# wangg12/mx-DeepIM

Measured on AMD Instinct MI355X. Metric: pose-refinements/sec (4 iters, 480x640), higher is better.
Workload: dtype f32

## Files before the change

### include/deepim_hip.h

```cpp
#ifndef DEEPIM_HIP_H_
#define DEEPIM_HIP_H_

#ifdef __cplusplus
extern "C" {
#endif

#define DIM_OK 0
#define DIM_ERR_ARG (-1)
#define DIM_ERR_LAUNCH (-2)
#define DIM_STATUS_OBS_BOX_EMPTY 1
#define DIM_STATUS_REN_BOX_EMPTY 2
#define DIM_STATUS_BAD_CLASS 4
#define DIM_STATUS_BAD_FACE 8
#define DIM_STATUS_BAD_K 16
#define DIM_STATUS_ICP_FEW_POINTS 32
#define DIM_STATUS_HYP_NO_SCORE 64
#define DIM_STATUS_FLOW_PNP_FEW_POINTS 128
#define DIM_STATUS_LAYER_HIDDEN 256
#define DIM_STATUS_COARSE_BAD_BOX 512
#define DIM_STATUS_PHOTO_FEW_POINTS 1024
#define DIM_STATUS_SIL_FEW_POINTS 2048
#define DIM_STATUS_TRACK_LOST 4096
#define DIM_STATUS_TRACK_REINIT 8192
#define DIM_STATUS_TRACK_OCCLUDED 16384
// ... 239 lines not shown

int dim_modelnet_light_position(const float* poses, float dx, float dy, float dz, float* light_pos, int B, void* stream);
int dim_box_mask(const int* bbox, float* mask, int B, int H, int W, int* bbox_of_mask, void* stream);

long dim_scene_compose_workspace_bytes(int N, int S, int H, int W);
int dim_scene_compose(const float* layer_bgr, const float* layer_depth, const int* layer_label, int N, int S, int H, int W,
                      void* workspace, float* scene_bgr, float* scene_depth, float* scene_label, float* vis_mask, int* counts,
                      int* vis_bbox, int* status, void* stream);

long dim_conv2d_packed_weight_floats(int Cout, int Cin, int KH, int KW);
int dim_conv2d_pack_weight(const float* w_oihw, float* w_packed, int Cout, int Cin, int KH, int KW, void* stream);
long dim_conv2d_workspace_floats(int N, int H, int W, int Cin, int Cout, int KH, int KW, int stride, int pad, int splits);
int dim_conv2d_fwd(const float* x, const float* w_packed, const float* bias, float* y, float* workspace, int N, int H, int W,
                   int Cin, int Cout, int KH, int KW, int stride, int pad, float slope, int splits, int tile, void* stream);
int dim_conv2d_fwd_partial(const float* x, const float* w_packed, float* workspace, int N, int H, int W, int Cin, int Cout, int KH,
                           int KW, int stride, int pad, int splits, int tile, void* stream);
int dim_splitk_reduce(const float* slabs, const float* bias, float* y, long M, int Cout, int splits, float slope, void* stream);
int dim_conv2d_tail_plan(int M, int Cout, int Cin, int KH, int KW, int tile, int* tail_begin_tile, int* tail_splits);
int dim_conv_auto_plan(long M, int Cout, int nchunks, int cin, int* tile, int* splits);
int dim_winograd_gemm_tile(int Cout, long tiles);
int dim_winograd_gemm_tile_planes(int Cout, long tiles, int planes);
int dim_set_winograd_split(int on);
int dim_get_winograd_split(void);
long dim_winograd_plane_gemm_weight_floats(int K, int Cout, int P);
int dim_winograd_plane_gemm_split_weights(float* U_packed, int K, int Cout, int P, void* stream);
int dim_winograd_plane_gemm(const float* V, const float* U_packed, float* M, int T, int K, int Cout, int P, int tile, int* used_split,
                            void* stream);
int dim_conv2d_fwd_ex(const float* x, const float* w_packed, const float* bias, float* y, int N, int H, int W, int Cin, int in_cstride,
                      int Cout, int KH, int KW, int stride, int pad, float slope, int tile, int out_cstride, int out_coff, int OH,
                      int OW, int osy, int osx, int ooy, int oox, int Ho, int Wo, int pad_w, int accumulate, void* stream);

long dim_winograd_packed_weight_floats(int Cout, int Cin, int m);
long dim_winograd_workspace_floats(int N, int H, int W, int Cin, int Cout, int m);
int dim_winograd_pack_weight(const float* w_oihw, float* w_packed, int Cout, int Cin, int m, void* stream);
int dim_winograd_dgrad_pack_weight(const float* w_oihw, float* w_packed, int Cout, int Cin, int m, void* stream);
int dim_conv2d_fwd_winograd(const float* x, const float* w_packed, const float* bias, float* y, float* workspace, int N, int H, int W,
                            int Cin, int in_cstride, int Cout, int out_cstride, int out_coff, float slope, int tile, int m,
                            void** events4, void* stream);
long dim_winograd5x5s2_packed_weight_floats(int Cout, int Cin);
long dim_winograd5x5s2_workspace_floats(int N, int H, int W, int Cin, int Cout);
int dim_winograd5x5s2_pack_weight(const float* w_oihw, float* w_packed, int Cout, int Cin, void* stream);
int dim_conv2d_fwd_winograd5x5s2(const float* x, const float* w_packed, const float* bias, float* y, float* workspace, int N, int H, int W,
                                 int Cin, int in_cstride, int Cout, int out_cstride, int out_coff, float slope, int tile, void** events4,
                                 void* stream);
int dim_wino_item_map_create(void** map, int N, int H, int W, int Cin, int Cout, int tile);
void dim_wino_item_map_destroy(void* map);
// ... 176 lines not shown
```

### mx-deepim_amd/csrc/common.h

```cpp
#pragma once
#include <hip/hip_runtime.h>
#include <cstdarg>
#include <cstdio>
#include <cstdint>
#include <utility>

#include "../../include/deepim_hip.h"

namespace dim {

constexpr int kWave = 64;

char* err_buf();
int set_err(int code, const char* fmt, ...);

inline hipStream_t as_stream(void* s) { return reinterpret_cast<hipStream_t>(s); }

inline int check_launch(const char* what) {
  hipError_t e = hipGetLastError();
  if (e != hipSuccess) return set_err(DIM_ERR_LAUNCH, "%s: %s", what, hipGetErrorString(e));
  return DIM_OK;
}

inline int ceil_div(long a, long b) { return (int)((a + b - 1) / b); }
// ... 177 lines not shown
int conv2d_unpack_weight_slabs(const float* w_packed, int nslab, long slab_stride, float* w_oihw, int Cout, int CoutPad, int Cin, int KH, int KW,
                               float scale, int accumulate, void* stream);

struct WGemmArgs {
  const float* V;
  const float* U;
  float* M;
  int T, K, Cout, P;
  int nch;
  int NTN;
  int per, rem;
  unsigned v_bytes, u_bytes, m_bytes;
  FastDiv d_nch, d_P, d_NTN, d_MT;
  int G, BM, BN, tile;
  int MT;
  int plane_major;
  int dbg_plain;
  int wide_flush;
  const void* U3;
  unsigned u3_bytes;
  int split;
  int skip5, q;
  const int* sigma;
};
inline long wino_packed_with_split(long u_floats) { return u_floats + (u_floats * 3 + 1) / 2; }
int wino_split_weights(float* U, long chunks, int Cout, hipStream_t st);
void wino_set_split(int on);
int wino_get_split();
bool wino_gemm_split_has(int tile);
int wino_gemm_split_slots(int tile);
int wino_gemm_split_run(const WGemmArgs& a, hipStream_t st);
int wino_gemm_plan(WGemmArgs* plan, const float* V, const float* U, float* M, int T, int K, int Cout, int P, int tile, int skip5 = 0);
void wino_tile_shape(int* tile, int Cout, int* BM, int* BN);
enum { kMapT, kMapK, kMapCout, kMapTile, kMapG, kMapPer, kMapRem, kMapLiveBefore, kMapLiveAfter, kMapMoved, kMapItems, kMapNch, kMapWords };
struct WinoItemMap {
  int hdr[kMapWords];
  int* host;
  int* dev;
};
int wino_item_map_build(int T, int K, int Cout, int tile, int G, int skip5, int* hdr, int** table);
inline const int* wino_item_map_for(const WinoItemMap* m, const WGemmArgs& a) {
  if (!m || !m->dev || !a.split || !a.skip5) return nullptr;
  const int* h = m->hdr;
  return (h[kMapT] == a.T && h[kMapK] == a.K && h[kMapCout] == a.Cout && h[kMapTile] == a.tile && h[kMapG] == a.G && h[kMapPer] == a.per &&
          h[kMapRem] == a.rem) ? m->dev : nullptr;
}
int wino_gemm_run(const WGemmArgs& plan, bool zeroed, hipStream_t st);

#ifdef __HIPCC__
struct WCur {
  int ch, p, nt, mt;
  int m;
// ... 123 lines not shown
```

### mx-deepim_amd/csrc/conv.hip

```cpp
#include "conv_impl.h"

namespace dim {

__global__ void splitk_reduce_kernel(const float* __restrict__ slabs, const float* __restrict__ bias, float* __restrict__ y,
                                     long MC, int Cout, int splits, float slope, int has_bias) {
  long i4 = (long)blockIdx.x * blockDim.x + threadIdx.x;
  long i = i4 * 4;
  if (i >= MC) return;
  float4 s = *reinterpret_cast<const float4*>(slabs + i);
  for (int k = 1; k < splits; ++k) {
    float4 p = *reinterpret_cast<const float4*>(slabs + (long)k * MC + i);
    s.x += p.x; s.y += p.y; s.z += p.z; s.w += p.w;
  }
  if (has_bias) {
    int c = (int)(i % Cout);
    s.x += bias[c]; s.y += bias[c + 1]; s.z += bias[c + 2]; s.w += bias[c + 3];
  }
  s.x = s.x > 0.f ? s.x : s.x * slope;
  s.y = s.y > 0.f ? s.y : s.y * slope;
  s.z = s.z > 0.f ? s.z : s.z * slope;
  s.w = s.w > 0.f ? s.w : s.w * slope;
  *reinterpret_cast<float4*>(y + i) = s;
}

// ... 84 lines not shown
  auto best_split = [&](long tiles, int smax) {
    double best = 1e30;
    int bs = 1;
    for (int s = 1; s <= smax; ++s) {
      if (!(s * 4 <= nchunks || s == 1)) continue;
      const double t = (double)((tiles * s + n_cu - 1) / n_cu) / s + 0.02 * s;
      if (t < best) { best = t; bs = s; }
    }
    return bs;
  };
  const bool wide = Cout % 128 == 0 && cin != 8;
  const long tiles = wide ? (M + 127) / 128 * (Cout / 128) : (M + 63) / 64 * (Cout / 64);
  *tile = wide ? 4 : 3;
  *splits = tiles >= n_cu ? 0 : best_split(tiles, 8);
  return DIM_OK;
}

int dim_set_winograd_split(int on) {
  wino_set_split(on ? 1 : 0);
  return DIM_OK;
}
int dim_get_winograd_split(void) { return wino_get_split(); }

static bool plane_gemm_on_device(const void* p) {
  hipPointerAttribute_t at;
  const hipError_t e = hipPointerGetAttributes(&at, p);
  if (e != hipSuccess) (void)hipGetLastError();
  return e == hipSuccess && (at.type == hipMemoryTypeDevice || at.type == hipMemoryTypeManaged);
}
long dim_winograd_plane_gemm_weight_floats(int K, int Cout, int P) {
  if (K <= 0 || Cout <= 0 || P <= 0) return 0;
  return wino_packed_with_split((long)P * K * Cout);
}
int dim_winograd_plane_gemm_split_weights(float* U_packed, int K, int Cout, int P, void* stream) {
  DIM_REQUIRE(K > 0 && K % 32 == 0 && Cout > 0 && Cout % 64 == 0 && P > 0, "winograd plane gemm: K %% 32 == 0 and Cout %% 64 == 0 required");
  DIM_REQUIRE(U_packed, "null pointer");
  DIM_REQUIRE(plane_gemm_on_device(U_packed), "winograd plane gemm: U_packed is not a device pointer");
  return wino_split_weights(U_packed, (long)P * (K / 32), Cout, as_stream(stream));
}
int dim_winograd_plane_gemm(const float* V, const float* U_packed, float* M, int T, int K, int Cout, int P, int tile, int* used_split,
                            void* stream) {
  DIM_REQUIRE(T > 0 && K > 0 && K % 32 == 0 && Cout > 0 && Cout % 64 == 0 && P > 0,
              "winograd plane gemm: T, P > 0, K %% 32 == 0 and Cout %% 64 == 0 required");
  DIM_REQUIRE(V && U_packed && M && used_split, "null pointer");
  DIM_REQUIRE(plane_gemm_on_device(V) && plane_gemm_on_device(U_packed) && plane_gemm_on_device(M),
              "winograd plane gemm: V, U_packed and M must be device pointers");
  WGemmArgs plan;
  const int rc = wino_gemm_plan(&plan, V, U_packed, M, T, K, Cout, P, tile);
  if (rc != DIM_OK) return rc;
  *used_split = plan.split;
  return wino_gemm_run(plan, false, as_stream(stream));
}

int dim_winograd_gemm_tile_planes(int Cout, long tiles, int planes) {
  static const int bn256 = [] { const char* e = getenv("DIM_WINO_BN256"); return e ? atoi(e) : 1; }();
  static const int fewrow = [] { const char* e = getenv("DIM_WINO_FEWROW"); return e ? atoi(e) : 1; }();
  if (Cout % 128) return 3;
  if (tiles < 1024) {
    if (!fewrow) return 3;
    if (wino_get_split()) {
      const struct { int tile, bm; double eff; } cand[2] = {{4, 128, 1.0}, {7, 96, planes > 36 ? 0.75 : 0.85}};
      const int cus = 256, slots = 512;
      int best = 7;
      double best_cost = 1e30;
      for (const auto& c : cand) {
        const long items = (tiles + c.bm - 1) / c.bm * (Cout / 128) * planes;
        long G = items < slots ? items : slots;
        if (G > cus && G < slots) G = G / cus * cus;
        const double cost = (double)items / (double)G * c.bm / c.eff;
        if (cost < best_cost) { best_cost = cost; best = c.tile; }
      }
      return best;
    }
    const struct { int tile, bm; double eff; } cand[3] = {{3, 64, 0.54}, {7, 96, 0.70}, {6, 160, 0.74}};
    int best = 3;
    double best_cost = 1e30;
    for (const auto& c : cand) {
      const double cost = (double)((tiles + c.bm - 1) / c.bm * c.bm) / c.eff;
      if (cost < best_cost) { best_cost = cost; best = c.tile; }
    }
    return best;
  }
  static const int big = [] { const char* e = getenv("DIM_WINO_BIG_TILE"); return e ? atoi(e) : 0; }();
  if (big == 6 || big == 7) return big;
  return (Cout % 256 == 0 && bn256) ? 5 : 4;
}
int dim_winograd_gemm_tile(int Cout, long tiles) { return dim_winograd_gemm_tile_planes(Cout, tiles, 36); }

// ... 359 lines not shown
```

### mx-deepim_amd/csrc/wino_gemm.hip

```cpp
#include <cstdlib>

#include "common.h"

namespace dim {

typedef float f32x16 __attribute__((ext_vector_type(16)));

__device__ __forceinline__ void wcur_advance(WCur& c, const WGemmArgs& a) {
  if (a.plane_major) return wcur_advance_pm(c, a);
  if (++c.ch == a.nch) {
    c.ch = 0;
    if (a.plane_major) {
      if (++c.nt == a.NTN) {
        c.nt = 0;
        if (++c.mt == a.MT) {
          c.mt = 0;
          ++c.p;
        }
      }
    } else if (++c.p == a.P) {
      c.p = 0;
      if (++c.nt == a.NTN) {
        c.nt = 0;
        ++c.mt;
// ... 180 lines not shown
    W_MFMA_GROUP(1, SET, 3)                                                            \
    buf ^= 1;                                                                          \
    W_FLUSH_CHECK(KCUR)                                                                \
  }
  int buf = 0;
  for (int kc = c_begin; kc < c_end; kc += 2) {
    W_CHUNK_BODY(0, kc)
    if (kc + 1 < c_end) W_CHUNK_BODY(1, kc + 1)
  }
#undef W_CHUNK_BODY
#undef W_FLUSH_CHECK
#undef W_MFMA_GROUP
#undef W_LOAD_BFRAG
#undef W_FRAG_READ
#undef W_STORE_CHUNK
#undef W_LOAD_CHUNK
}

__global__ __launch_bounds__(256) void wino_gemm_zero_kernel(WGemmArgs a) { wino_gemm_zero_tile(a, blockIdx.x + 1); }

static int g_wino_split = getenv("DIM_WINO_SPLIT") ? atoi(getenv("DIM_WINO_SPLIT")) : 1;
void wino_set_split(int on) { g_wino_split = on; }
int wino_get_split() { return g_wino_split; }
static int g_wino_cus = 0;
template <int BM, int BN, int WM, int WN>
static int wino_gemm_slots() {
  static int slots = 0;
  if (slots == 0) {
    int dev = 0, cus = 0, occ = 0;
    hipError_t e = hipGetDevice(&dev);
    if (e == hipSuccess) e = hipDeviceGetAttribute(&cus, hipDeviceAttributeMultiprocessorCount, dev);
    if (e == hipSuccess)
      e = hipOccupancyMaxActiveBlocksPerMultiprocessor(&occ, reinterpret_cast<const void*>(&wino_gemm_kernel<BM, BN, WM, WN>),
                                                       WM * WN * 64, (2 * BM * 36 + WM * WN * 512) * sizeof(float));
    if (e != hipSuccess || cus <= 0 || occ <= 0) return set_err(DIM_ERR_LAUNCH, "winograd gemm occupancy query: %s", hipGetErrorString(e));
    slots = cus * occ;
    g_wino_cus = cus;
  }
  return slots;
}

void wino_tile_shape(int* tile, int Cout, int* BM, int* BN) {
  if (*tile == 5 && Cout % 256 != 0) *tile = 4;
  if ((*tile < 4 || *tile > 7) || Cout % 128 != 0) *tile = 3;
  *BM = *tile == 3 ? 64 : *tile == 6 ? 160 : *tile == 7 ? 96 : 128;
  *BN = *tile == 5 ? 256 : *tile == 3 ? 64 : 128;
// ... 18 lines not shown
  a.P = P;
  a.nch = K / 32;
  a.NTN = Cout / BN;
  a.v_bytes = (unsigned)((long)T * P * K * 4);
  a.u_bytes = (unsigned)((long)P * K * Cout * 4);
  a.m_bytes = (unsigned)((long)T * P * Cout * 4);
  a.d_nch = make_fastdiv((unsigned)a.nch);
  a.d_P = make_fastdiv((unsigned)P);
  a.d_NTN = make_fastdiv((unsigned)a.NTN);
  a.MT = (int)MT;
  a.d_MT = make_fastdiv((unsigned)MT);
  static const int order = getenv("DIM_WINO_PLANE_MAJOR") ? atoi(getenv("DIM_WINO_PLANE_MAJOR")) : 1;
  a.plane_major = order;
  static const int dbg_plain = getenv("DIM_WINO_DBG_PLAIN") ? atoi(getenv("DIM_WINO_DBG_PLAIN")) : 0;
  a.dbg_plain = dbg_plain;
  static const int wide = getenv("DIM_WINO_WIDE_FLUSH") ? atoi(getenv("DIM_WINO_WIDE_FLUSH")) : 1;
  a.wide_flush = wide;
  a.BM = BM;
  a.BN = BN;
  a.tile = tile;
  a.split = g_wino_split && wino_gemm_split_has(tile) && (long)P * K * Cout * 6 < (1L << 31);
  a.U3 = U + (long)P * K * Cout;
  a.u3_bytes = (unsigned)((long)P * K * Cout * 6);
  DIM_REQUIRE(!skip5 || (P == 36 && a.nch % 4 == 0), "winograd gemm: skipping zero phase blocks needs 36 planes and K = 4 phases of whole chunks");
  a.skip5 = skip5;
  a.q = a.nch / 4;
  if (a.split || skip5) a.plane_major = 1;
  const int slots = a.split ? wino_gemm_split_slots(tile) : tile == 5 ? wino_gemm_slots<128, 256, 2, 4>() : tile == 4 ? wino_gemm_slots<128, 128, 2, 4>()
                  : tile == 6 ? wino_gemm_slots<160, 128, 1, 4>() : tile == 7 ? wino_gemm_slots<96, 128, 1, 4>() : wino_gemm_slots<64, 64, 2, 2>();
  if (slots <= 0) return slots;
  a.G = items < slots ? (int)items : slots;
  static const int g_round = getenv("DIM_WINO_G_ROUND") ? atoi(getenv("DIM_WINO_G_ROUND")) : 1;
  if (g_wino_cus == 0) {
    int dev = 0;
    if (hipGetDevice(&dev) != hipSuccess || hipDeviceGetAttribute(&g_wino_cus, hipDeviceAttributeMultiprocessorCount, dev) != hipSuccess) g_wino_cus = 0;
  }
  if (g_round && g_wino_cus > 0 && a.G > g_wino_cus && a.G < slots) a.G = a.G / g_wino_cus * g_wino_cus;
  if (const char* e = getenv("DIM_WINO_MAX_G")) {
    const int cap = atoi(e);
    if (cap > 0 && cap < a.G) a.G = cap;
  }
  const long total = items * a.nch;
  a.per = (int)(total / a.G);
  a.rem = (int)(total % a.G);
  *plan = a;
  return DIM_OK;
// ... 29 lines not shown
```

### mx-deepim_amd/csrc/wino_gemm_split.hip

```cpp
#include <cstdlib>

#include "common.h"

#ifndef DIM_SPLIT_EXP
#define DIM_SPLIT_EXP 0
#endif
#ifndef DIM_SPLIT_OPT
#define DIM_SPLIT_OPT 0
#endif

namespace dim {

typedef float f32x16 __attribute__((ext_vector_type(16)));
typedef float f32x4 __attribute__((ext_vector_type(4)));
typedef __bf16 bf16x8 __attribute__((ext_vector_type(8)));
typedef __bf16 bf16x4 __attribute__((ext_vector_type(4)));

struct Split4 {
  uint2 h, m, l;
};
__device__ __forceinline__ Split4 split3(const float4 v) {
  const f32x4 x = {v.x, v.y, v.z, v.w};
  const bf16x4 bh = __builtin_convertvector(x, bf16x4);
  const f32x4 r1 = x - __builtin_convertvector(bh, f32x4);
// ... 31 lines not shown
                     make_fastdiv((unsigned)Cout));
  return check_launch("winograd_split_weights");
}

#if DIM_SPLIT_EXP & 128
__device__ unsigned long long g_split_stamps[1024 * 8 * 11];
#endif
#if (DIM_SPLIT_EXP & 128) && defined(__HIP_DEVICE_COMPILE__)
#define S_STAMP(K)                                                                     \
  {                                                                                    \
    unsigned long long t_;                                                             \
    __builtin_amdgcn_sched_barrier(0);                                                 \
    asm volatile("s_memtime %0\n\ts_waitcnt lgkmcnt(0)" : "=s"(t_)::"memory");         \
    __builtin_amdgcn_sched_barrier(0);                                                 \
    seg[K] += t_ - tprev;                                                              \
    tprev = t_;                                                                        \
  }
#else
#define S_STAMP(K)
#endif

__device__ __forceinline__ void wscur_advance(WCur& c, const WGemmArgs& a, const WTab& t) { wcur_advance_pm(c, a, t); }

template <int BM, int WN, bool TAB>
__device__ __forceinline__ void wino_gemm_split_body(const WGemmArgs& a) {
  constexpr int BK = 32;
  constexpr int NT = WN * 64;
  constexpr int BN = 32 * WN;
  constexpr int TM = BM / 32;
  constexpr int RP = NT / 8;
  constexpr int NSTG = BM / RP;
  constexpr int PL = BM * 64;
  constexpr int kTrLd = 32, kTrFloats = 16 * kTrLd;
  constexpr int kMAux = ((DIM_SPLIT_OPT & 2) || BM == 96) ? 0 : 2;
  static_assert(BM % 32 == 0 && BM % RP == 0 && RP % 32 == 0 && NSTG >= 2 && NSTG <= 4, "two to four staging loads per thread");

  extern __shared__ __attribute__((aligned(16))) unsigned char smem_split[];
  unsigned char* sA = smem_split;
  float* sTr = reinterpret_cast<float*>(smem_split + 2 * 3 * PL);

  const int tid = threadIdx.x;
  const int lane = tid & 63;
  const int wave = tid >> 6;
  const int q = tid & 7;
  const int srow = tid >> 3;
  const int frow = lane & 31;
  const int khalf = lane >> 5;

  const int wg = wg_xcd_contiguous(blockIdx.x, a.G);
  const int r_begin = wg_first_chunk(wg, a);
  const WTab tab = TAB ? wtab_load(r_begin, a) : WTab{0, 0, false};
  const int c_begin = 0, c_end = wcur_count(r_begin, wg_first_chunk(wg + 1, a), a, tab);
  if (c_end == 0) return;

  const int RS = a.P * a.K;
  const int a_voff0 = (srow * RS + q * 4) * 4;
  const int a_vstep = RP * RS * 4;
  const __amdgpu_buffer_rsrc_t rv = __builtin_amdgcn_make_buffer_rsrc(const_cast<float*>(a.V), 0, a.v_bytes, 0x00020000);
  const __amdgpu_buffer_rsrc_t ru = __builtin_amdgcn_make_buffer_rsrc(const_cast<void*>(a.U3), 0, a.u3_bytes, 0x00020000);
  const __amdgpu_buffer_rsrc_t rm = __builtin_amdgcn_make_buffer_rsrc(a.M, 0, a.m_bytes, 0x00020000);
  const int wchunk_bytes = a.Cout * 192;

  WCur L = wcur_decode(r_begin, a, tab), Bc = L, C = L;

  float4 rav[2][NSTG];
#define S_LOAD_PREP(PF_OK)                                                             \
  const bool l_pf = (PF_OK);                                                           \
  const int l_mb = L.mt * BM;                                                          \
  const int l_soff = (int)((unsigned)(l_mb * RS + L.p * a.K + L.ch * BK) * 4u);        \
  wscur_advance(L, a, tab);
#define S_LOAD_ISSUE(RSET)                                                             \
  _Pragma("unroll") for (int ps = 0; ps < NSTG; ++ps)                                   \
    rav[RSET][ps] = buf_load16_nt(rv, (l_pf && l_mb + srow + ps * RP < a.T) ? a_voff0 + ps * a_vstep : -1, l_soff);
  const int st_off = srow * 64 + ((((q >> 1) ^ (srow >> 2)) & 3) << 4) + (q & 1) * 8;
#define S_STORE_ONE(DA, R, PASS)                                                       \
  {                                                                                    \
    const Split4 s = split3(R);                                                        \
    *reinterpret_cast<uint2*>((DA) + (PASS) * RP * 64) = s.h;                          \
    *reinterpret_cast<uint2*>((DA) + PL + (PASS) * RP * 64) = s.m;                     \
    *reinterpret_cast<uint2*>((DA) + 2 * PL + (PASS) * RP * 64) = s.l;                 \
  }
#define S_STORE_CHUNK(BUF, RSET)                                                       \
  {                                                                                    \
    unsigned char* dA = sA + (BUF) * 3 * PL + st_off;                                  \
    _Pragma("unroll") for (int ps = 0; ps < NSTG; ++ps) S_STORE_ONE(dA, rav[RSET][ps], ps) \
  }

  f32x16 acc[TM];
#pragma unroll
  for (int i = 0; i < TM; ++i)
#pragma unroll
    for (int r = 0; r < 16; ++r) acc[i][r] = 0.f;

  const int fr_off = frow * 64 + (((khalf ^ (frow >> 2)) & 3) << 4);
  bf16x8 fa[TM][3];
#define S_FRAG_READ(T, PA, S)                                                                                          \
  {                                                                                                                    \
    _Pragma("unroll") for (int i = 0; i < TM; ++i)                                                                      \
      fa[i][T] = *reinterpret_cast<const bf16x8*>((PA) + (T) * PL + i * 2048 + (fr_off ^ (32 * (S))));                 \
  }
  bf16x8 fb[2][3][2];
  const int bf_voff = wave * 6144 + frow * 32 + khalf * 16;
#define S_BFRAG_PREP(VALID)                                                                                            \
  const int b_soff = (VALID) ? (Bc.p * a.nch + Bc.ch) * wchunk_bytes + Bc.nt * BN * 192 : 0;                            \
  wscur_advance(Bc, a, tab);
#define S_BFRAG_ISSUE(SET)                                                                                             \
  _Pragma("unroll") for (int t = 0; t < 3; ++t) _Pragma("unroll") for (int s = 0; s < 2; ++s) {                         \
    const float4 v = buf_load16(ru, bf_voff + (t * 2 + s) * 1024, b_soff);                                             \
    fb[SET][t][s] = __builtin_bit_cast(bf16x8, v);                                                                     \
  }
  static constexpr int kTA[2][6] = {{2, 0, 1, 1, 0, 0}, {2, 1, 1, 0, 0, 0}};
  static constexpr int kTB[2][6] = {{0, 2, 1, 0, 1, 0}, {0, 1, 0, 2, 1, 0}};
  f32x4 sp_x, sp_r;
  bf16x4 sp_h, sp_m, sp_l;

  const int ldc = a.P * a.Cout;
  const int o_row = 4 * khalf;
  const int o_col = wave * 32 + frow;
  const int o_voff = (o_row * ldc + o_col) * 4;
  bool whole = C.ch == 0;
#define S_FLUSH_CHECK(KCUR)                                                                                            \
  {                                                                                                                    \
    const bool item_end = wcur_item_end(C, a);                                                                         \
    if (item_end || (KCUR) == c_end - 1) {                                                                             \
      const int mb = C.mt * BM;                                                                                        \
      const int cb = C.p * a.Cout + C.nt * BN;                                                                         \
      const int lim = a.T - mb;                                                                                        \
      int ov = o_voff, orow = o_row;                                                                                   \
      asm volatile("" : "+v"(ov), "+v"(orow));                                                                         \
      const int soff = (int)((unsigned)(mb * ldc + cb) * 4u);                                                          \
      const bool plain = (whole && item_end) || a.dbg_plain;                                                           \
      if (plain && a.wide_flush) {                                                                                     \
        float* sT = sTr + wave * kTrFloats;                                                                            \
        const int trow = lane >> 3, tc4 = (lane & 7) * 4;                                                              \
        _Pragma("unroll") for (int i = 0; i < TM; ++i) _Pragma("unroll") for (int h = 0; h < 2; ++h) {                  \
                \
          if constexpr (!(DIM_SPLIT_OPT & 16))                                                                         \
// ... 19 lines not shown
            __builtin_amdgcn_raw_buffer_store_b128(u1, rm, vo1, soff, kMAux);                                          \
          }                                                                                                            \
        }                                                                                                              \
      } else                                                                                                           \
      _Pragma("unroll") for (int i = 0; i < TM; ++i) _Pragma("unroll") for (int r = 0; r < 16; ++r) {                   \
        const int dr = 32 * i + (r & 3) + 8 * (r >> 2);                                                                \
        const int vo = (orow + dr < lim) ? ov + dr * ldc * 4 : -1;                                                     \
        if (plain)                                                                                                     \
          __builtin_amdgcn_raw_buffer_store_b32(__float_as_uint(acc[i][r]), rm, vo, soff, 2);                          \
        else if (vo != -1)                                                                                             \
          __builtin_amdgcn_raw_ptr_buffer_atomic_fadd_f32(acc[i][r], rm, vo, soff, 0);                                 \
      }                                                                                                                \
      if constexpr (!(DIM_SPLIT_OPT & 32))                                                                             \
      _Pragma("unroll") for (int i = 0; i < TM; ++i) _Pragma("unroll") for (int r = 0; r < 16; ++r) acc[i][r] = 0.f;    \
      whole = true;                                                                                                    \
    }                                                                                                                  \
    wscur_advance(C, a, tab);                                                                                               \
  }

  {
    S_LOAD_PREP(true)
    S_LOAD_ISSUE(0)
  }
  S_STORE_CHUNK(0, 0)
  {
    S_BFRAG_PREP(true)
    S_BFRAG_ISSUE(0)
  }
  {
    S_LOAD_PREP(c_begin + 1 < c_end)
    S_LOAD_ISSUE(1)
  }
  {
    S_LOAD_PREP(c_begin + 2 < c_end)
    S_LOAD_ISSUE(0)
  }
  __syncthreads();

#define S_CHUNK_BODY(SET, KCUR)                                                        \
  {                                                                                    \
    const unsigned char* cA = sA + buf * 3 * PL;                                       \
    unsigned char* dA = sA + (buf ^ 1) * 3 * PL + st_off;                              \
    S_BFRAG_PREP((KCUR) + 1 < c_end)                                                   \
    S_LOAD_PREP((KCUR) + 3 < c_end)                                                    \
    __builtin_amdgcn_sched_barrier(0);                                                 \
    if constexpr (!(DIM_SPLIT_EXP & 16)) {                                             \
      S_FRAG_READ(2, cA, 0)                                                            \
      S_FRAG_READ(0, cA, 0)                                                            \
      S_FRAG_READ(1, cA, 0)                                                            \
    }                                                                                  \
    if constexpr (!(DIM_SPLIT_EXP & 4)) S_BFRAG_ISSUE(1 - SET)                         \
    __builtin_amdgcn_sched_barrier(0);                                                 \
    static_for<12 * TM>([&](auto N_) {                                                 \
      constexpr int n = decltype(N_)::value;                                           \
      constexpr int ks = n / (6 * TM), ti = (n % (6 * TM)) / TM, i = n % TM;           \
      constexpr int TA = kTA[ks][ti], TB = kTB[ks][ti];                                \
      if constexpr (!(DIM_SPLIT_EXP & 1))                                              \
        acc[i] = __builtin_amdgcn_mfma_f32_32x32x16_bf16(fa[i][TA], fb[SET][TB][ks], acc[i], 0, 0, 0); \
      else {                                                                           \
        asm volatile("" ::"v"(fa[i][TA]));                                             \
        asm volatile("" ::"v"(fb[SET][TB][ks]));                                       \
      }                                                                                \
                          \
      if constexpr (n < 6 * NSTG && !(DIM_SPLIT_EXP & 8)) {                            \
        constexpr int ps = n / 6, sub = n % 6;                                         \
        if constexpr (sub == 0) {                                                      \
          const float4 v = rav[1 - SET][ps];                                           \
          sp_x = f32x4{v.x, v.y, v.z, v.w};                                            \
          sp_h = __builtin_convertvector(sp_x, bf16x4);                                \
        } else if constexpr (sub == 1) {                                               \
          sp_r = sp_x - __builtin_convertvector(sp_h, f32x4);                          \
        } else if constexpr (sub == 2) {                                               \
          sp_m = __builtin_convertvector(sp_r, bf16x4);                                \
        } else if constexpr (sub == 3) {                                               \
          sp_r = sp_r - __builtin_convertvector(sp_m, f32x4);                          \
        } else if constexpr (sub == 4) {                                               \
          sp_l = __builtin_convertvector(sp_r, bf16x4);                                \
        } else {                                                                       \
          *reinterpret_cast<uint2*>(dA + ps * RP * 64) = __builtin_bit_cast(uint2, sp_h);          \
          *reinterpret_cast<uint2*>(dA + PL + ps * RP * 64) = __builtin_bit_cast(uint2, sp_m);     \
          *reinterpret_cast<uint2*>(dA + 2 * PL + ps * RP * 64) = __builtin_bit_cast(uint2, sp_l); \
        }                                                                              \
      }                                                                                \
       \
      if constexpr (!(DIM_SPLIT_EXP & 16)) {                                           \
        if constexpr (n >= 2 * TM && n < 3 * TM)                                       \
          fa[n - 2 * TM][2] = *reinterpret_cast<const bf16x8*>(cA + 2 * PL + (n - 2 * TM) * 2048 + (fr_off ^ 32)); \
        if constexpr (n >= 3 * TM && n < 4 * TM)                                       \
          fa[n - 3 * TM][1] = *reinterpret_cast<const bf16x8*>(cA + PL + (n - 3 * TM) * 2048 + (fr_off ^ 32));     \
        if constexpr (n >= 5 * TM && n < 6 * TM)                                       \
          fa[n - 5 * TM][0] = *reinterpret_cast<const bf16x8*>(cA + (n - 5 * TM) * 2048 + (fr_off ^ 32));          \
      }                                                                                \
        \
      if constexpr (n >= 6 * TM && (n - 6 * TM) % 2 == 0 && (n - 6 * TM) / 2 < NSTG && !(DIM_SPLIT_EXP & 2)) { \
        constexpr int ps = (n - 6 * TM) / 2;                                           \
        rav[1 - SET][ps] = buf_load16_nt(rv, (l_pf && l_mb + srow + ps * RP < a.T) ? a_voff0 + ps * a_vstep : -1, l_soff); \
      }                                                                                \
      __builtin_amdgcn_sched_barrier(0);                                               \
    });                                                                                \
    S_STAMP(0)                                                                         \
    if constexpr (!(DIM_SPLIT_EXP & 64)) S_FLUSH_CHECK(KCUR) else wscur_advance(C, a, tab); \
    S_STAMP(1)                                                                         \
    if constexpr (!(DIM_SPLIT_EXP & 32)) asm volatile("s_waitcnt lgkmcnt(0)\n\ts_barrier" ::: "memory"); \
    S_STAMP(2)                                                                         \
    buf ^= 1;                                                                          \
  }
  int buf = 0;
#if (DIM_SPLIT_EXP & 128) && defined(__HIP_DEVICE_COMPILE__)
  unsigned long long seg[8] = {0, 0, 0, 0, 0, 0, 0, 0}, tprev, tstart;
  asm volatile("s_memtime %0\n\ts_waitcnt lgkmcnt(0)" : "=s"(tprev)::"memory");
  tstart = tprev;
#endif
  for (int kc = c_begin; kc < c_end; kc += 2) {
    S_CHUNK_BODY(0, kc)
    if (kc + 1 < c_end) S_CHUNK_BODY(1, kc + 1)
  }
#if (DIM_SPLIT_EXP & 64) && defined(__HIP_DEVICE_COMPILE__)
  _Pragma("unroll") for (int i = 0; i < TM; ++i) asm volatile("" ::"v"(acc[i]));
#endif
#if (DIM_SPLIT_EXP & 128) && defined(__HIP_DEVICE_COMPILE__)
  if (lane == 0 && blockIdx.x < 1024 && wave < 8) {
    unsigned long long* o = g_split_stamps + (blockIdx.x * 8 + wave) * 11;
    for (int k = 0; k < 8; ++k) o[k] = seg[k];
    o[8] = tprev - tstart;
    o[9] = (unsigned long long)(c_end - c_begin);
    o[10] = 1;
  }
#endif
#undef S_CHUNK_BODY
#undef S_FLUSH_CHECK
#undef S_BFRAG_ISSUE
#undef S_BFRAG_PREP
#undef S_FRAG_READ
#undef S_STORE_CHUNK
#undef S_STORE_ONE
#undef S_LOAD_ISSUE
#undef S_LOAD_PREP
}

template <int BM, int WN>
__global__ __launch_bounds__(WN * 64) __attribute__((amdgpu_waves_per_eu(2, 2))) void wino_gemm_split_kernel(WGemmArgs a) {
  wino_gemm_split_body<BM, WN, false>(a);
}
template <int BM, int WN>
__global__ __launch_bounds__(WN * 64) __attribute__((amdgpu_waves_per_eu(2, 2))) void wino_gemm_split_map_kernel(WGemmArgs a) {
  wino_gemm_split_body<BM, WN, true>(a);
}

template <int BM, int WN>
static constexpr size_t split_lds_bytes() {
  return 2 * 3 * BM * 64 + WN * 16 * 32 * sizeof(float);
}

template <int BM, int WN>
static int wino_gemm_split_slots_t() {
  static int slots = 0;
  if (slots == 0) {
    int dev = 0, cus = 0, occ = 0;
    hipError_t e = hipGetDevice(&dev);
    if (e == hipSuccess) e = hipDeviceGetAttribute(&cus, hipDeviceAttributeMultiprocessorCount, dev);
    if (e == hipSuccess)
      e = hipOccupancyMaxActiveBlocksPerMultiprocessor(&occ, reinterpret_cast<const void*>(&wino_gemm_split_kernel<BM, WN>), WN * 64,
                                                       split_lds_bytes<BM, WN>());
    if (e != hipSuccess || cus <= 0 || occ <= 0) return set_err(DIM_ERR_LAUNCH, "winograd split gemm occupancy query: %s", hipGetErrorString(e));
    slots = cus * occ;
  }
  return slots;
}

bool wino_gemm_split_has(int tile) { return tile == 5 || tile == 4 || tile == 7; }

int wino_gemm_split_slots(int tile) {
  return tile == 5 ? wino_gemm_split_slots_t<128, 8>() : tile == 4 ? wino_gemm_split_slots_t<128, 4>() : wino_gemm_split_slots_t<96, 4>();
}

template <int BM, int WN>
static int wino_gemm_split_launch(const WGemmArgs& a, hipStream_t st) {
  constexpr size_t lds = split_lds_bytes<BM, WN>();
  static_assert(lds <= 65536, "a workgroup's dynamic LDS stays within 64 KB (see wino_gemm.hip)");
  if (a.sigma)
    hipLaunchKernelGGL((wino_gemm_split_map_kernel<BM, WN>), dim3(a.G), dim3(WN * 64), lds, st, a);
  else
    hipLaunchKernelGGL((wino_gemm_split_kernel<BM, WN>), dim3(a.G), dim3(WN * 64), lds, st, a);
  return check_launch("winograd_gemm_split");
}

#if DIM_SPLIT_EXP & 128
extern "C" int dim_debug_split_stamps(unsigned long long* host, int n) {
  return (int)hipMemcpyFromSymbol(host, HIP_SYMBOL(g_split_stamps), sizeof(unsigned long long) * 11 * 8 * (n < 1024 ? n : 1024));
}
#endif

int wino_gemm_split_run(const WGemmArgs& a, hipStream_t st) {
  if (a.tile == 5) return wino_gemm_split_launch<128, 8>(a, st);
  if (a.tile == 4) return wino_gemm_split_launch<128, 4>(a, st);
  return wino_gemm_split_launch<96, 4>(a, st);
}

}
```

### mx-deepim_amd/lib/hip/capi.py

```python
import ctypes
import os

import numpy as np

_HERE = os.path.dirname(os.path.abspath(__file__))
LIB_PATH = os.environ.get("DIM_HIP_LIB") or os.path.normpath(os.path.join(_HERE, "..", "libdeepim_hip.so"))

P = ctypes.c_void_p
I = ctypes.c_int
F = ctypes.c_float
L = ctypes.c_long
D = ctypes.c_double

SIGNATURES = {
    "dim_last_error": (ctypes.c_char_p, []),
    "dim_device_info": (I, [ctypes.c_char_p, I]),
    "dim_mask_bbox": (I, [P, I, I, I, I, I, F, P, P, P]),
    "dim_zoom_factor": (I, [P, P, P, P, I, I, I, P, P, P]),
    "dim_zoom_planes": (I, [P, P, P, I, I, I, I, I, I, I, P, I, P]),
    "dim_zoom_net_input": (I, [P, P, P, P, P, P, I, I, I, P, P, P, P, P, P]),
    "dim_zoom_net_input_ex": (I, [P, P, P, P, P, P, I, I, I, P, I, P]),
    "dim_zoom_planes_src": (I, [P, P, P, I, I, I, I, I, I, I, I, P, P]),
    "dim_zoom_net_input_src": (I, [P, P, P, P, P, P, I, I, I, I, I, P, I, P, P, P, P, P]),
    "dim_zoom_planes_area": (I, [P, P, P, I, I, I, I, I, I, I, I, P, I, P]),
# ... 106 lines not shown
    "dim_fc_unpack_weight": (I, [P, P, I, I, I, I, P]),
    "dim_fc_dgrad_pack_weight": (I, [P, P, I, I, I, I, P]),
    "dim_flow_loss_grad": (I, [P, P, P, P, L, F, F, P, P]),
    "dim_logistic_grad": (I, [P, P, P, P, L, F, P]),
    "dim_pm_l1_grad": (I, [P, P, P, P, L, F, F, P, P]),
    "dim_pm_loss_grad": (I, [P, P, P, P, L, F, F, I, F, P, P]),
    "dim_pm_sym_workspace_bytes": (L, [I, I, I]),
    "dim_pm_sym_loss_grad": (I, [P, P, P, P, P, P, I, P, I, I, I, F, F, I, F, P, P, P, P, P, P, P]),
    "dim_se3_dist_loss_grad": (I, [P, P, P, P, P, P, P, P, I, F, F, I, F, P, P]),
    "dim_quat_normalize": (I, [P, P, I, P]),
    "dim_pose_head_bwd": (I, [P, P, P, P, P, P, P, P, P, P, P, I, P]),
    "dim_fc_wgrad": (I, [P, P, P, P, I, I, I, P]),
    "dim_fc_wgrad_nhwc": (I, [P, P, P, I, I, I, I, I, P]),
    "dim_upsample16_bwd": (I, [P, P, P, I, I, I, I, I, I, I, F, P]),
    "dim_conv_small_cout_bwd_workspace_floats": (L, [I, I, I, I, I, I, I]),
    "dim_conv_small_cout_bwd": (I, [P, P, P, P, P, P, P, I, I, I, I, I, I, I, I, I, I, I, P]),
    "dim_deconv4x4s2_tiny_bwd": (I, [P, I, P, I, I, P, P, P, P, I, I, I, I, I, I, I, I, P]),
    "dim_conv2d_tail_plan": (I, [I, I, I, I, I, I, P, P]),
    "dim_conv_auto_plan": (I, [L, I, I, I, P, P]),
    "dim_winograd_gemm_tile": (I, [I, L]),
    "dim_winograd_gemm_tile_planes": (I, [I, L, I]),
    "dim_set_winograd_split": (I, [I]),
    "dim_get_winograd_split": (I, []),
    "dim_winograd_plane_gemm_weight_floats": (L, [I, I, I]),
    "dim_winograd_plane_gemm_split_weights": (I, [P, I, I, I, P]),
    "dim_winograd_plane_gemm": (I, [P, P, P, I, I, I, I, I, P, P]),
    "dim_winograd_packed_weight_floats": (L, [I, I, I]),
    "dim_winograd_workspace_floats": (L, [I, I, I, I, I, I]),
    "dim_winograd_pack_weight": (I, [P, P, I, I, I, P]),
    "dim_winograd_dgrad_pack_weight": (I, [P, P, I, I, I, P]),
    "dim_winograd3x3s2_packed_weight_floats": (L, [I, I]),
    "dim_winograd3x3s2_use": (I, [I, I, I, I]),
    "dim_winograd3x3s2_workspace_floats": (L, [I, I, I, I, I]),
    "dim_winograd3x3s2_pack_weight": (I, [P, P, I, I, P]),
    "dim_conv2d_fwd_winograd3x3s2": (I, [P, P, P, P, P, I, I, I, I, I, I, I, I, F, I, P, P]),
    "dim_winograd5x5s2_packed_weight_floats": (L, [I, I]),
    "dim_winograd5x5s2_workspace_floats": (L, [I, I, I, I, I]),
    "dim_winograd5x5s2_pack_weight": (I, [P, P, I, I, P]),
    "dim_conv2d_fwd_winograd5x5s2": (I, [P, P, P, P, P, I, I, I, I, I, I, I, I, F, I, P, P]),
    "dim_wino_item_map_create": (I, [P, I, I, I, I, I, I]),
    "dim_wino_item_map_destroy": (None, [P]),
    "dim_wino_item_map_query": (I, [P, P, P, L]),
    "dim_wino_item_map_plan": (I, [I, I, I, I, I, I, P, P, L]),
    "dim_conv2d_fwd_winograd5x5s2_map": (I, [P, P, P, P, P, I, I, I, I, I, I, I, I, F, I, P, P, P]),
    "dim_winograd5x5s2_dgrad_pack_weight": (I, [P, P, I, I, P]),
    "dim_conv2d_dgrad_winograd5x5s2": (I, [P, P, P, P, I, I, I, I, I, I, I, I, P]),
# ... 103 lines not shown
```

### mx-deepim_amd/lib/hip/ops.py

```python
import struct

import numpy as np

import torch

from . import capi
from .capi import check, current_stream, dptr, host_f32, lib

f32 = torch.float32
i32 = torch.int32
bf16 = torch.bfloat16


def to_bf16(src, out=None):
    out = out if out is not None else torch.empty(src.shape, dtype=bf16, device=src.device)
    check(lib().dim_f32_to_bf16(dptr(src, f32), dptr(out, bf16), src.numel(), current_stream()))
    return out


def from_bf16(src, out=None):
    out = out if out is not None else torch.empty(src.shape, dtype=f32, device=src.device)
    check(lib().dim_bf16_to_f32(dptr(src, bf16), dptr(out, f32), src.numel(), current_stream()))
    return out

# ... 1149 lines not shown
    check(lib().dim_fill_words(dptr(dst), dst.numel(), bits, current_stream()))
    return dst


def copy_channels(dst_oihw, dst_c0, src_oihw, src_c0, nch):
    O, Id, kh, kw = dst_oihw.shape
    Os, Is = src_oihw.shape[:2]
    assert O == Os and tuple(src_oihw.shape[2:]) == (kh, kw) and dst_oihw.is_contiguous() and src_oihw.is_contiguous()
    assert 0 <= dst_c0 and dst_c0 + nch <= Id and 0 <= src_c0 and src_c0 + nch <= Is
    t = kh * kw
    check(lib().dim_copy_rows(dptr(dst_oihw, f32) + 4 * dst_c0 * t, Id * t, dptr(src_oihw, f32) + 4 * src_c0 * t, Is * t, O, nch * t,
                              current_stream()))
    return dst_oihw


def set_winograd_split(on):
    check(lib().dim_set_winograd_split(1 if on else 0))


def get_winograd_split():
    return bool(lib().dim_get_winograd_split())


def winograd_plane_gemm(V, U_pkn, T, K, Cout, P, tile, out=None):
    import ctypes

    assert tuple(V.shape) == (T, P, K) and tuple(U_pkn.shape) == (P, K, Cout) and K % 32 == 0, (V.shape, U_pkn.shape)
    n = P * K * Cout
    wp = _new((lib().dim_winograd_plane_gemm_weight_floats(K, Cout, P),), V)
    wp[:n] = U_pkn.reshape(P, K // 32, 32, Cout).permute(0, 1, 3, 2).reshape(-1)
    check(lib().dim_winograd_plane_gemm_split_weights(dptr(wp, f32), K, Cout, P, current_stream()))
    out = out if out is not None else _new((T, P, Cout), V)
    used = ctypes.c_int(-1)
    check(lib().dim_winograd_plane_gemm(dptr(V, f32), dptr(wp, f32), dptr(out, f32), T, K, Cout, P, int(tile), ctypes.byref(used),
                                        current_stream()))
    return out, used.value


def winograd_pack_weight(w_oihw, m=2):
    Cout, Cin, KH, KW = w_oihw.shape
    assert KH == 3 and KW == 3
    out = _new((lib().dim_winograd_packed_weight_floats(Cout, Cin, m),), w_oihw)
    check(lib().dim_winograd_pack_weight(dptr(w_oihw, f32), dptr(out, f32), Cout, Cin, m, current_stream()))
    return out


# ... 601 lines not shown
```

Baseline: 1739.

## Stream f32 Winograd weights and split to bf16 terms in-kernel for few-row GEMMs

```diff
diff --git a/include/deepim_hip.h b/include/deepim_hip.h
--- a/include/deepim_hip.h
+++ b/include/deepim_hip.h
@@ -285,6 +285,9 @@
 int dim_winograd_gemm_tile_planes(int Cout, long tiles, int planes);
 int dim_set_winograd_split(int on);
 int dim_get_winograd_split(void);
+int dim_set_winograd_weight_stream(int mode);
+int dim_get_winograd_weight_stream(void);
+int dim_winograd_plane_gemm_weight_stream(int T, int K, int Cout, int P, int tile);
 long dim_winograd_plane_gemm_weight_floats(int K, int Cout, int P);
 int dim_winograd_plane_gemm_split_weights(float* U_packed, int K, int Cout, int P, void* stream);
 int dim_winograd_plane_gemm(const float* V, const float* U_packed, float* M, int T, int K, int Cout, int P, int tile, int* used_split,
diff --git a/mx-deepim_amd/csrc/common.h b/mx-deepim_amd/csrc/common.h
--- a/mx-deepim_amd/csrc/common.h
+++ b/mx-deepim_amd/csrc/common.h
@@ -223,12 +223,16 @@
   int split;
   int skip5, q;
   const int* sigma;
+  int wstream;
 };
 inline long wino_packed_with_split(long u_floats) { return u_floats + (u_floats * 3 + 1) / 2; }
 int wino_split_weights(float* U, long chunks, int Cout, hipStream_t st);
 void wino_set_split(int on);
 int wino_get_split();
 bool wino_gemm_split_has(int tile);
+bool wino_gemm_split_has_f32w(int tile);
+void wino_set_weight_stream(int mode);
+int wino_get_weight_stream();
 int wino_gemm_split_slots(int tile);
 int wino_gemm_split_run(const WGemmArgs& a, hipStream_t st);
 int wino_gemm_plan(WGemmArgs* plan, const float* V, const float* U, float* M, int T, int K, int Cout, int P, int tile, int skip5 = 0);
diff --git a/mx-deepim_amd/csrc/conv.hip b/mx-deepim_amd/csrc/conv.hip
--- a/mx-deepim_amd/csrc/conv.hip
+++ b/mx-deepim_amd/csrc/conv.hip
@@ -130,6 +130,18 @@
 }
 int dim_get_winograd_split(void) { return wino_get_split(); }
 
+int dim_set_winograd_weight_stream(int mode) {
+  DIM_REQUIRE(mode >= 0 && mode <= 2, "winograd weight stream: mode 0, 1 or 2");
+  wino_set_weight_stream(mode);
+  return DIM_OK;
+}
+int dim_get_winograd_weight_stream(void) { return wino_get_weight_stream(); }
+int dim_winograd_plane_gemm_weight_stream(int T, int K, int Cout, int P, int tile) {
+  WGemmArgs plan;
+  const int rc = wino_gemm_plan(&plan, nullptr, nullptr, nullptr, T, K, Cout, P, tile);
+  return rc != DIM_OK ? rc : plan.wstream;
+}
+
 static bool plane_gemm_on_device(const void* p) {
   hipPointerAttribute_t at;
   const hipError_t e = hipPointerGetAttributes(&at, p);
@@ -168,10 +180,12 @@
     if (!fewrow) return 3;
     if (wino_get_split()) {
       const struct { int tile, bm; double eff; } cand[2] = {{4, 128, 1.0}, {7, 96, planes > 36 ? 0.75 : 0.85}};
-      const int cus = 256, slots = 512;
+      const int cus = device_cu_count();
       int best = 7;
       double best_cost = 1e30;
       for (const auto& c : cand) {
+        int slots = wino_gemm_split_slots(c.tile);
+        if (slots <= 0) slots = 2 * cus;
         const long items = (tiles + c.bm - 1) / c.bm * (Cout / 128) * planes;
         long G = items < slots ? items : slots;
         if (G > cus && G < slots) G = G / cus * cus;
diff --git a/mx-deepim_amd/csrc/wino_gemm.hip b/mx-deepim_amd/csrc/wino_gemm.hip
--- a/mx-deepim_amd/csrc/wino_gemm.hip
+++ b/mx-deepim_amd/csrc/wino_gemm.hip
@@ -226,6 +226,10 @@
 static int g_wino_split = getenv("DIM_WINO_SPLIT") ? atoi(getenv("DIM_WINO_SPLIT")) : 1;
 void wino_set_split(int on) { g_wino_split = on; }
 int wino_get_split() { return g_wino_split; }
+static int g_wino_weight_stream = 1;
+constexpr int kWStreamMaxRowTiles = 2;
+void wino_set_weight_stream(int mode) { g_wino_weight_stream = mode; }
+int wino_get_weight_stream() { return g_wino_weight_stream; }
 static int g_wino_cus = 0;
 template <int BM, int BN, int WM, int WN>
 static int wino_gemm_slots() {
@@ -290,6 +294,8 @@
   a.split = g_wino_split && wino_gemm_split_has(tile) && (long)P * K * Cout * 6 < (1L << 31);
   a.U3 = U + (long)P * K * Cout;
   a.u3_bytes = (unsigned)((long)P * K * Cout * 6);
+  a.wstream = a.split && wino_gemm_split_has_f32w(tile) && !skip5 &&
+              (g_wino_weight_stream == 2 || (g_wino_weight_stream == 1 && MT <= kWStreamMaxRowTiles));
   DIM_REQUIRE(!skip5 || (P == 36 && a.nch % 4 == 0), "winograd gemm: skipping zero phase blocks needs 36 planes and K = 4 phases of whole chunks");
   a.skip5 = skip5;
   a.q = a.nch / 4;
diff --git a/mx-deepim_amd/csrc/wino_gemm_split.hip b/mx-deepim_amd/csrc/wino_gemm_split.hip
--- a/mx-deepim_amd/csrc/wino_gemm_split.hip
+++ b/mx-deepim_amd/csrc/wino_gemm_split.hip
@@ -77,9 +77,12 @@
 
 __device__ __forceinline__ void wscur_advance(WCur& c, const WGemmArgs& a, const WTab& t) { wcur_advance_pm(c, a, t); }
 
-template <int BM, int WN, bool TAB>
+template <int BM, int WN, bool TAB, bool F32W>
 __device__ __forceinline__ void wino_gemm_split_body(const WGemmArgs& a) {
   constexpr int BK = 32;
+  constexpr bool kF32W = F32W;
+  constexpr int kWColBytes = kF32W ? 128 : 192;
+  static_assert(!(TAB && kF32W), "the f32 weight stream has no item-slot table");
   constexpr int NT = WN * 64;
   constexpr int BN = 32 * WN;
   constexpr int TM = BM / 32;
@@ -112,9 +115,10 @@
   const int a_voff0 = (srow * RS + q * 4) * 4;
   const int a_vstep = RP * RS * 4;
   const __amdgpu_buffer_rsrc_t rv = __builtin_amdgcn_make_buffer_rsrc(const_cast<float*>(a.V), 0, a.v_bytes, 0x00020000);
-  const __amdgpu_buffer_rsrc_t ru = __builtin_amdgcn_make_buffer_rsrc(const_cast<void*>(a.U3), 0, a.u3_bytes, 0x00020000);
+  const __amdgpu_buffer_rsrc_t ru = kF32W ? __builtin_amdgcn_make_buffer_rsrc(const_cast<float*>(a.U), 0, a.u_bytes, 0x00020000)
+                                          : __builtin_amdgcn_make_buffer_rsrc(const_cast<void*>(a.U3), 0, a.u3_bytes, 0x00020000);
   const __amdgpu_buffer_rsrc_t rm = __builtin_amdgcn_make_buffer_rsrc(a.M, 0, a.m_bytes, 0x00020000);
-  const int wchunk_bytes = a.Cout * 192;
+  const int wchunk_bytes = a.Cout * kWColBytes;
 
   WCur L = wcur_decode(r_begin, a, tab), Bc = L, C = L;
 
@@ -154,20 +158,38 @@
     _Pragma("unroll") for (int i = 0; i < TM; ++i)                                                                      \
       fa[i][T] = *reinterpret_cast<const bf16x8*>((PA) + (T) * PL + i * 2048 + (fr_off ^ (32 * (S))));                 \
   }
-  bf16x8 fb[2][3][2];
-  const int bf_voff = wave * 6144 + frow * 32 + khalf * 16;
+  u32x4 fb[2][3][2];
+  float4 ub[4];
+  const int bf_voff = kF32W ? (wave * 32 + frow) * 128 + khalf * 32 : wave * 6144 + frow * 32 + khalf * 16;
 #define S_BFRAG_PREP(VALID)                                                                                            \
-  const int b_soff = (VALID) ? (Bc.p * a.nch + Bc.ch) * wchunk_bytes + Bc.nt * BN * 192 : 0;                            \
+  const int b_soff = (VALID) ? (Bc.p * a.nch + Bc.ch) * wchunk_bytes + Bc.nt * BN * kWColBytes : 0;                     \
   wscur_advance(Bc, a, tab);
 #define S_BFRAG_ISSUE(SET)                                                                                             \
   _Pragma("unroll") for (int t = 0; t < 3; ++t) _Pragma("unroll") for (int s = 0; s < 2; ++s) {                         \
     const float4 v = buf_load16(ru, bf_voff + (t * 2 + s) * 1024, b_soff);                                             \
-    fb[SET][t][s] = __builtin_bit_cast(bf16x8, v);                                                                     \
+    fb[SET][t][s] = __builtin_bit_cast(u32x4, v);                                                                      \
+  }
+#define S_BRAW_ISSUE()                                                                                                 \
+  _Pragma("unroll") for (int j = 0; j < 4; ++j) ub[j] = buf_load16(ru, bf_voff + (j >> 1) * 64 + (j & 1) * 16, b_soff);
+#define S_BTERMS_PUT(SET, J, H, M, L)                                                                                  \
+  {                                                                                                                    \
+    const uint2 h_ = (H), m_ = (M), l_ = (L);                                                                          \
+    if constexpr (((J) & 1) == 0) {                                                                                    \
+      fb[SET][0][(J) >> 1].x = h_.x; fb[SET][0][(J) >> 1].y = h_.y;                                                    \
+      fb[SET][1][(J) >> 1].x = m_.x; fb[SET][1][(J) >> 1].y = m_.y;                                                    \
+      fb[SET][2][(J) >> 1].x = l_.x; fb[SET][2][(J) >> 1].y = l_.y;                                                    \
+    } else {                                                                                                           \
+      fb[SET][0][(J) >> 1].z = h_.x; fb[SET][0][(J) >> 1].w = h_.y;                                                    \
+      fb[SET][1][(J) >> 1].z = m_.x; fb[SET][1][(J) >> 1].w = m_.y;                                                    \
+      fb[SET][2][(J) >> 1].z = l_.x; fb[SET][2][(J) >> 1].w = l_.y;                                                    \
+    }                                                                                                                  \
   }
   static constexpr int kTA[2][6] = {{2, 0, 1, 1, 0, 0}, {2, 1, 1, 0, 0, 0}};
   static constexpr int kTB[2][6] = {{0, 2, 1, 0, 1, 0}, {0, 1, 0, 2, 1, 0}};
   f32x4 sp_x, sp_r;
   bf16x4 sp_h, sp_m, sp_l;
+  f32x4 bs_r;
+  bf16x4 bs_h, bs_m;
 
   const int ldc = a.P * a.Cout;
   const int o_row = 4 * khalf;
@@ -233,10 +255,20 @@
     S_LOAD_PREP(true)
     S_LOAD_ISSUE(0)
   }
+  if constexpr (kF32W) {
+    S_BFRAG_PREP(true)
+    S_BRAW_ISSUE()
+  }
   S_STORE_CHUNK(0, 0)
-  {
+  if constexpr (!kF32W) {
     S_BFRAG_PREP(true)
     S_BFRAG_ISSUE(0)
+  } else {
+    static_for<4>([&](auto J_) {
+      constexpr int j = decltype(J_)::value;
+      const Split4 s = split3(ub[j]);
+      S_BTERMS_PUT(0, j, s.h, s.m, s.l)
+    });
   }
   {
     S_LOAD_PREP(c_begin + 1 < c_end)
@@ -260,14 +292,20 @@
       S_FRAG_READ(0, cA, 0)                                                            \
       S_FRAG_READ(1, cA, 0)                                                            \
     }                                                                                  \
-    if constexpr (!(DIM_SPLIT_EXP & 4)) S_BFRAG_ISSUE(1 - SET)                         \
+    if constexpr (!(DIM_SPLIT_EXP & 4)) {                                              \
+      if constexpr (!kF32W) {                                                          \
+        S_BFRAG_ISSUE(1 - SET)                                                         \
+      } else {                                                                         \
+        S_BRAW_ISSUE()                                                                 \
+      }                                                                                \
+    }                                                                                  \
     __builtin_amdgcn_sched_barrier(0);                                                 \
     static_for<12 * TM>([&](auto N_) {                                                 \
       constexpr int n = decltype(N_)::value;                                           \
       constexpr int ks = n / (6 * TM), ti = (n % (6 * TM)) / TM, i = n % TM;           \
       constexpr int TA = kTA[ks][ti], TB = kTB[ks][ti];                                \
       if constexpr (!(DIM_SPLIT_EXP & 1))                                              \
-        acc[i] = __builtin_amdgcn_mfma_f32_32x32x16_bf16(fa[i][TA], fb[SET][TB][ks], acc[i], 0, 0, 0); \
+        acc[i] = __builtin_amdgcn_mfma_f32_32x32x16_bf16(fa[i][TA], __builtin_bit_cast(bf16x8, fb[SET][TB][ks]), acc[i], 0, 0, 0); \
       else {                                                                           \
         asm volatile("" ::"v"(fa[i][TA]));                                             \
         asm volatile("" ::"v"(fb[SET][TB][ks]));                                       \
@@ -302,6 +340,21 @@
         if constexpr (n >= 5 * TM && n < 6 * TM)                                       \
           fa[n - 5 * TM][0] = *reinterpret_cast<const bf16x8*>(cA + (n - 5 * TM) * 2048 + (fr_off ^ 32));          \
       }                                                                                \
+       \
+      if constexpr (kF32W && n >= 12 * TM - 8) {                                       \
+        constexpr int g = n - (12 * TM - 8), j = g >> 1;                               \
+        if constexpr ((g & 1) == 0) {                                                  \
+          const float4 v = ub[j];                                                      \
+          const f32x4 x = {v.x, v.y, v.z, v.w};                                        \
+          bs_h = __builtin_convertvector(x, bf16x4);                                   \
+          bs_r = x - __builtin_convertvector(bs_h, f32x4);                             \
+          bs_m = __builtin_convertvector(bs_r, bf16x4);                                \
+        } else {                                                                       \
+          bs_r = bs_r - __builtin_convertvector(bs_m, f32x4);                          \
+          const bf16x4 bs_l = __builtin_convertvector(bs_r, bf16x4);                   \
+          S_BTERMS_PUT(1 - SET, j, __builtin_bit_cast(uint2, bs_h), __builtin_bit_cast(uint2, bs_m), __builtin_bit_cast(uint2, bs_l)) \
+        }                                                                              \
+      }                                                                                \
         \
       if constexpr (n >= 6 * TM && (n - 6 * TM) % 2 == 0 && (n - 6 * TM) / 2 < NSTG && !(DIM_SPLIT_EXP & 2)) { \
         constexpr int ps = (n - 6 * TM) / 2;                                           \
@@ -340,6 +393,8 @@
 #endif
 #undef S_CHUNK_BODY
 #undef S_FLUSH_CHECK
+#undef S_BTERMS_PUT
+#undef S_BRAW_ISSUE
 #undef S_BFRAG_ISSUE
 #undef S_BFRAG_PREP
 #undef S_FRAG_READ
@@ -351,11 +406,15 @@
 
 template <int BM, int WN>
 __global__ __launch_bounds__(WN * 64) __attribute__((amdgpu_waves_per_eu(2, 2))) void wino_gemm_split_kernel(WGemmArgs a) {
-  wino_gemm_split_body<BM, WN, false>(a);
+  wino_gemm_split_body<BM, WN, false, false>(a);
 }
 template <int BM, int WN>
 __global__ __launch_bounds__(WN * 64) __attribute__((amdgpu_waves_per_eu(2, 2))) void wino_gemm_split_map_kernel(WGemmArgs a) {
-  wino_gemm_split_body<BM, WN, true>(a);
+  wino_gemm_split_body<BM, WN, true, false>(a);
+}
+template <int BM, int WN>
+__global__ __launch_bounds__(WN * 64) __attribute__((amdgpu_waves_per_eu(2, 2))) void wino_gemm_split_f32w_kernel(WGemmArgs a) {
+  wino_gemm_split_body<BM, WN, false, true>(a);
 }
 
 template <int BM, int WN>
@@ -380,6 +439,7 @@
 }
 
 bool wino_gemm_split_has(int tile) { return tile == 5 || tile == 4 || tile == 7; }
+bool wino_gemm_split_has_f32w(int tile) { return tile == 4 || tile == 7; }
 
 int wino_gemm_split_slots(int tile) {
   return tile == 5 ? wino_gemm_split_slots_t<128, 8>() : tile == 4 ? wino_gemm_split_slots_t<128, 4>() : wino_gemm_split_slots_t<96, 4>();
@@ -391,7 +451,12 @@
   static_assert(lds <= 65536, "a workgroup's dynamic LDS stays within 64 KB (see wino_gemm.hip)");
   if (a.sigma)
     hipLaunchKernelGGL((wino_gemm_split_map_kernel<BM, WN>), dim3(a.G), dim3(WN * 64), lds, st, a);
-  else
+  else if (a.wstream) {
+    if constexpr (WN == 4)
+      hipLaunchKernelGGL((wino_gemm_split_f32w_kernel<BM, WN>), dim3(a.G), dim3(WN * 64), lds, st, a);
+    else
+      return set_err(DIM_ERR_ARG, "winograd split gemm: tile %d has no f32 weight stream", a.tile);
+  } else
     hipLaunchKernelGGL((wino_gemm_split_kernel<BM, WN>), dim3(a.G), dim3(WN * 64), lds, st, a);
   return check_launch("winograd_gemm_split");
 }
diff --git a/mx-deepim_amd/lib/hip/capi.py b/mx-deepim_amd/lib/hip/capi.py
--- a/mx-deepim_amd/lib/hip/capi.py
+++ b/mx-deepim_amd/lib/hip/capi.py
@@ -152,6 +152,9 @@
     "dim_winograd_gemm_tile_planes": (I, [I, L, I]),
     "dim_set_winograd_split": (I, [I]),
     "dim_get_winograd_split": (I, []),
+    "dim_set_winograd_weight_stream": (I, [I]),
+    "dim_get_winograd_weight_stream": (I, []),
+    "dim_winograd_plane_gemm_weight_stream": (I, [I, I, I, I, I]),
     "dim_winograd_plane_gemm_weight_floats": (L, [I, I, I]),
     "dim_winograd_plane_gemm_split_weights": (I, [P, I, I, I, P]),
     "dim_winograd_plane_gemm": (I, [P, P, P, I, I, I, I, I, P, P]),
diff --git a/mx-deepim_amd/lib/hip/ops.py b/mx-deepim_amd/lib/hip/ops.py
--- a/mx-deepim_amd/lib/hip/ops.py
+++ b/mx-deepim_amd/lib/hip/ops.py
@@ -1195,6 +1195,20 @@
     return bool(lib().dim_get_winograd_split())
 
 
+def set_winograd_weight_stream(mode):
+    check(lib().dim_set_winograd_weight_stream(int(mode)))
+
+
+def get_winograd_weight_stream():
+    return int(lib().dim_get_winograd_weight_stream())
+
+
+def winograd_plane_gemm_weight_stream(T, K, Cout, P, tile):
+    r = int(lib().dim_winograd_plane_gemm_weight_stream(int(T), int(K), int(Cout), int(P), int(tile)))
+    check(min(r, 0))
+    return r
+
+
 def winograd_plane_gemm(V, U_pkn, T, K, Cout, P, tile, out=None):
     import ctypes
 
```

New measurement: 1737 (median of 2 runs). No clear change (-0.2%).
